# bioinfomaticsCSU/deepsignal

Hardware: AMD Instinct MI355X
Metric: CpG sites/sec (batch=512, k=17, sig=360) (higher is better)
Workload: dtype f32; 1 GPU; configs[1]: 1xMI355X, batch=512, random-init CpG model weights, synthetic (17,360) features, fp32; batch=512, kmer_len=17, signal_len=360

## Files before the change

### deepsignal_amd/csrc/ds_device.h

```cpp
#pragma once
#include "ds_internal.h"

namespace ds {

typedef float floatx16 __attribute__((ext_vector_type(16)));

__device__ __forceinline__ float4 f4max(float4 a, float4 b)
{
    return make_float4(fmaxf(a.x, b.x), fmaxf(a.y, b.y), fmaxf(a.z, b.z), fmaxf(a.w, b.w));
}
__device__ __forceinline__ float sigmoidf_(float x) { return 1.0f / (1.0f + expf(-x)); }
__device__ __forceinline__ float fast_sigmoid(float x) { return __builtin_amdgcn_rcpf(1.0f + __expf(-x)); }
__device__ __forceinline__ float fast_tanh(float x) { return fmaf(2.0f, fast_sigmoid(2.0f * x), -1.0f); }

typedef float v4f __attribute__((ext_vector_type(4)));
typedef const __attribute__((address_space(1))) v4f* gptr4;
typedef const __attribute__((address_space(1))) float* gptr1;
typedef __attribute__((address_space(1))) float* gptr1w;
__device__ __forceinline__ float4 gload4(const float* p)
{
    const v4f v = *(gptr4)(p);
    return make_float4(v.x, v.y, v.z, v.w);
}
__device__ __forceinline__ float gload(const float* p) { return *(gptr1)(p); }
__device__ __forceinline__ float4 gload4_nt(const float* p)
{
    const v4f v = __builtin_nontemporal_load((gptr4)(p));
    return make_float4(v.x, v.y, v.z, v.w);
}
__device__ __forceinline__ void gstore(float* p, float v) { *(gptr1w)(p) = v; }

typedef __bf16 bf16x8 __attribute__((ext_vector_type(8)));
__device__ __forceinline__ float bf2max(float a, float b)
{
    const unsigned ua = __float_as_uint(a), ub = __float_as_uint(b);
    const float lo = fmaxf(__uint_as_float(ua << 16), __uint_as_float(ub << 16));
    const float hi = fmaxf(__uint_as_float(ua & 0xffff0000u), __uint_as_float(ub & 0xffff0000u));
    return __uint_as_float((__float_as_uint(hi) & 0xffff0000u) | (__float_as_uint(lo) >> 16));
}
__device__ __forceinline__ float4 bf8max(float4 a, float4 b)
{
    return make_float4(bf2max(a.x, b.x), bf2max(a.y, b.y), bf2max(a.z, b.z), bf2max(a.w, b.w));
}
typedef short short2v __attribute__((ext_vector_type(2)));
__device__ __forceinline__ float bf2max_nn(float a, float b)
{
    return __builtin_bit_cast(float, __builtin_elementwise_max(__builtin_bit_cast(short2v, a), __builtin_bit_cast(short2v, b)));
}
__device__ __forceinline__ float4 bf8max_nn(float4 a, float4 b)
{
    return make_float4(bf2max_nn(a.x, b.x), bf2max_nn(a.y, b.y), bf2max_nn(a.z, b.z), bf2max_nn(a.w, b.w));
}
__device__ __forceinline__ unsigned short f2bf(float v)
{
    return __builtin_bit_cast(unsigned short, (__bf16)v);
}
__device__ __forceinline__ float bf2f(unsigned short b) { return __uint_as_float((unsigned)b << 16); }
__device__ __forceinline__ float relu_f(float x)
{
    const int b = __builtin_bit_cast(int, x);
    return __builtin_bit_cast(float, b > 0 ? b : 0);
}
typedef __bf16 bf16x2_t __attribute__((ext_vector_type(2)));
typedef float float2_t __attribute__((ext_vector_type(2)));
__device__ __forceinline__ unsigned pack_bf2(float a, float b)
{
    const float2_t f = {a, b};
    return __builtin_bit_cast(unsigned, __builtin_convertvector(f, bf16x2_t));
}

__device__ __forceinline__ floatx16 mfma_bf(float4 a, float4 b, floatx16 c)
{
    return __builtin_amdgcn_mfma_f32_32x32x16_bf16(__builtin_bit_cast(bf16x8, a), __builtin_bit_cast(bf16x8, b), c, 0, 0, 0);
}

__device__ __forceinline__ void glds16(const void* gsrc, unsigned lds_dst)
{
    unsigned keep;
    asm volatile("s_mov_b32 %0, m0\n\ts_mov_b32 m0, %2\n\ts_nop 0\n\tglobal_load_lds_dwordx4 %1, off\n\ts_mov_b32 m0, %0"
                 : "=&s"(keep)
                 : "v"(gsrc), "s"(lds_dst)
                 : "memory");
}

__device__ __forceinline__ void glds16s(const void* gbase, unsigned lane_off, unsigned lds_dst)
{
    unsigned keep;
    asm volatile("s_mov_b32 %0, m0\n\ts_mov_b32 m0, %3\n\ts_nop 0\n\tglobal_load_lds_dwordx4 %1, %2\n\ts_mov_b32 m0, %0"
// ... 82 lines not shown
```

### deepsignal_amd/csrc/ds_engine.cpp

```cpp
#include "../../include/deepsignal_hip.h"
#include "ds_internal.h"
#include "ds_extract.h"

#include <algorithm>
#include <cmath>
#include <cstdio>
#include <cstdlib>
#include <cstring>
#include <functional>
#include <map>
#include <string>
#include <vector>

using namespace ds;

namespace {

constexpr int VOCAB = 1024, EMB = 128, HID = 256, NLAYER = 3, NMOD = 11, INC_OUT = 240;
constexpr double BN_EPS = 1e-3;

thread_local std::string g_create_error;

void same_pad(int in, int k, int s, int* out, int* pl)
{
// ... 165 lines not shown

    float *stem1_w = nullptr, *stem1_b = nullptr;
    PackedGemm conv2, conv3;
    PackedGemm m_f1[NMOD];
    PackedGemm m_s1[NMOD], m_b1[NMOD], m_b3b[NMOD], m_b4b[NMOD], m_b5b[NMOD], m_b5c[NMOD];
    PackedGemm lstm_n[2][NLAYER];
    float* lstm_table[2] = {nullptr, nullptr};
    float* lstm_wfeat[2] = {nullptr, nullptr};
    PackedGemm fc1;
    float* fc2 = nullptr;
    float* w12f = nullptr;

    bool debug_keep_pool = false;
    const float* zero_seg = nullptr;
    unsigned long long* dbg_stamps = nullptr;
    unsigned long long* dbg_lstm = nullptr;
    std::vector<Stage> stages;
    KernelStat kstat[K_COUNT];
    std::vector<Slot> slots;
    Slot* cur = nullptr;
    unsigned next_slot = 0;
    int64_t plan_tick = 0;
    bool stages_done = false;
};

namespace {

int fail(ds_handle* h, int code, const std::string& msg)
{
    if (h) h->err = msg; else g_create_error = msg;
    return code;
}

#define HIPCHK(h, expr)                                                                                  \
    do {                                                                                                 \
        hipError_t e_ = (expr);                                                                          \
        if (e_ != hipSuccess) {                                                                          \
            (void)hipGetLastError();  \
            return fail(h, DS_ERR_HIP, std::string(#expr) + ": " + hipGetErrorString(e_));              \
        }                                                                                                \
    } while (0)

template <class T>
int dalloc(ds_handle* h, T** p, size_t count)
{
    void* q = nullptr;
    size_t bytes = std::max<size_t>(count * sizeof(T), 256);
    hipError_t e = hipMalloc(&q, bytes);
    if (e != hipSuccess) {
        (void)hipGetLastError();
        return fail(h, DS_ERR_NOMEM, std::string("hipMalloc: ") + hipGetErrorString(e));
    }
    h->allocs.push_back(q);
    *p = static_cast<T*>(q);
    return DS_OK;
}

int upload(ds_handle* h, float** dst, const std::vector<float>& v)
{
    int rc = dalloc(h, dst, v.size());
    if (rc) return rc;
    HIPCHK(h, hipMemcpy(*dst, v.data(), v.size() * sizeof(float), hipMemcpyHostToDevice));
    return DS_OK;
}

std::vector<float> pack_b(int K, int N, const std::function<float(int, int)>& w_in)
{
    const int Kp = (K + 31) / 32 * 32;
    auto w = [&](int k, int col) { return k < K ? w_in(k, col) : 0.0f; };
    const int ntiles = (N + 31) / 32, kg = Kp / 8;
    std::vector<float> out((size_t)ntiles * kg * 256, 0.0f);
    for (int nt = 0; nt < ntiles; ++nt)
        for (int g = 0; g < kg; ++g)
            for (int lane = 0; lane < 64; ++lane) {
                const int col = nt * 32 + (lane & 31);
                if (col >= N) continue;
                const int k0 = g * 8 + 4 * (lane >> 5);
                float* o = &out[(((size_t)nt * kg + g) * 64 + lane) * 4];
                for (int s = 0; s < 4; ++s) o[s] = w(k0 + s, col);
            }
    return out;
}

uint16_t f32_to_bf16(float f)
{
    uint32_t u;
    memcpy(&u, &f, 4);
    if ((u & 0x7fffffffu) > 0x7f800000u) return (uint16_t)((u >> 16) | 0x40);
    u += 0x7fffu + ((u >> 16) & 1);
    return (uint16_t)(u >> 16);
}

std::vector<float> pack_b_bf16(int K, int N, const std::function<float(int, int)>& w_in)
{
    const int Kp = (K + 63) / 64 * 64;
    const int ntiles = (N + 31) / 32, ks = Kp / 16;
    std::vector<uint16_t> out((size_t)ntiles * ks * 64 * 8, 0);
    for (int nt = 0; nt < ntiles; ++nt)
        for (int g = 0; g < ks; ++g)
            for (int lane = 0; lane < 64; ++lane) {
                const int col = nt * 32 + (lane & 31);
                if (col >= N) continue;
                const int k0 = g * 16 + 8 * (lane >> 5);
                uint16_t* o = &out[(((size_t)nt * ks + g) * 64 + lane) * 8];
                for (int q = 0; q < 8; ++q) o[q] = k0 + q < K ? f32_to_bf16(w_in(k0 + q, col)) : 0;
            }
    std::vector<float> raw(out.size() / 2);
    memcpy(raw.data(), out.data(), out.size() * 2);
    return raw;
}

std::vector<float> pack_b_split(int K, int N, const std::function<float(int, int)>& w_in)
{
    const int Kp = (K + 63) / 64 * 64;
    const int ntiles = (N + 31) / 32, ks = Kp / 16;
    std::vector<uint16_t> out((size_t)ntiles * ks * 3 * 64 * 8, 0);
    for (int nt = 0; nt < ntiles; ++nt)
        for (int g = 0; g < ks; ++g)
            for (int lane = 0; lane < 64; ++lane) {
                const int col = nt * 32 + (lane & 31);
                if (col >= N) continue;
                const int k0 = g * 16 + 8 * (lane >> 5);
                for (int q = 0; q < 8; ++q) {
                    if (k0 + q >= K) continue;
                    float r = w_in(k0 + q, col);
                    for (int t = 0; t < 3; ++t) {
                        const uint16_t b = f32_to_bf16(r);
                        out[((((size_t)nt * ks + g) * 3 + t) * 64 + lane) * 8 + q] = b;
                        uint32_t u = (uint32_t)b << 16;
                        float f;
                        memcpy(&f, &u, 4);
                        r -= f;
                    }
                }
            }
    std::vector<float> raw(out.size() / 2);
    memcpy(raw.data(), out.data(), out.size() * 2);
    return raw;
}

struct FoldedConv {
    int k, cin, cout;
    std::vector<float> w;
    std::vector<float> b;
};

const HostTensor* find(ds_handle* h, const std::string& name)
{
    auto it = h->host.find(name);
    return it == h->host.end() ? nullptr : &it->second;
}

int fold_conv(ds_handle* h, const std::string& scope, const std::string& conv, const std::string& bn, int k, int cin,
              int cout, FoldedConv* out)
{
    const HostTensor* ker = find(h, scope + "/" + conv + "/kernel");
    const HostTensor* beta = find(h, scope + "/" + bn + "/beta");
    const HostTensor* gamma = find(h, scope + "/" + bn + "/gamma");
    const HostTensor* mean = find(h, scope + "/" + bn + "/moving_mean");
    const HostTensor* var = find(h, scope + "/" + bn + "/moving_variance");
    if (!ker || !beta || !gamma || !mean || !var)
        return fail(h, DS_ERR_INVALID, "missing tensor(s) under " + scope + "/" + conv);
    if ((int64_t)ker->data.size() != (int64_t)k * cin * cout || (int)beta->data.size() != cout ||
        (int)gamma->data.size() != cout || (int)mean->data.size() != cout || (int)var->data.size() != cout)
        return fail(h, DS_ERR_INVALID, "bad shape for " + scope + "/" + conv + " (kernel or one of beta/gamma/moving_mean/moving_variance)");
    out->k = k; out->cin = cin; out->cout = cout;
    out->w.resize((size_t)k * cin * cout);
    out->b.resize(cout);
    std::vector<double> sc(cout);
    for (int c = 0; c < cout; ++c) {
        sc[c] = (double)gamma->data[c] / std::sqrt((double)var->data[c] + BN_EPS);
        out->b[c] = (float)((double)beta->data[c] - (double)mean->data[c] * sc[c]);
    }
    for (size_t r = 0; r < (size_t)k * cin; ++r)
        for (int c = 0; c < cout; ++c) out->w[r * cout + c] = (float)((double)ker->data[r * cout + c] * sc[c]);
    return DS_OK;
}

int upload_concat(ds_handle* h, const std::vector<const FoldedConv*>& parts, PackedGemm* pg, bool split_panel = false)
{
    const int K = parts[0]->k * parts[0]->cin;
    int N = 0;
    for (auto* p : parts) N += p->cout;
    std::vector<int> owner(N), local(N);
    int c0 = 0;
    for (size_t i = 0; i < parts.size(); ++i) {
        for (int c = 0; c < parts[i]->cout; ++c) { owner[c0 + c] = (int)i; local[c0 + c] = c; }
        c0 += parts[i]->cout;
    }
    auto wfun = [&](int k, int col) {
        const FoldedConv* p = parts[owner[col]];
        return p->w[(size_t)k * p->cout + local[col]];
    };
    std::vector<float> packed = h->bf16 ? pack_b_bf16(K, N, wfun) : pack_b(K, N, wfun);
    std::vector<float> bias((N + 31) / 32 * 32, 0.0f);
    for (int col = 0; col < N; ++col) bias[col] = parts[owner[col]]->b[local[col]];
    pg->K = h->bf16 ? (K + 1) / 2 : K; pg->N = N;
    int rc = upload(h, &pg->Bp, packed);
    if (rc) return rc;
    if (split_panel && (rc = upload(h, &pg->Bps, pack_b_split(K, N, wfun)))) return rc;
    return upload(h, &pg->bias, bias);
}

std::string mod_root(int n)
{
    char buf[128];
    snprintf(buf, sizeof buf, "modelsignalmincp_layer%d/modelsignalm%d", n, n);
    return buf;
}

int finalize_weights(ds_handle* h)
{
    int rc;
    if (h->is_cnn) {
    FoldedConv c1, c2, c3;
    if ((rc = fold_conv(h, "modelsignalmconv_layer1", "conv", "bn", 7, 1, 64, &c1))) return rc;
    if ((rc = fold_conv(h, "modelsignalmconv_layer2", "conv", "bn", 1, 64, 128, &c2))) return rc;
    if ((rc = fold_conv(h, "modelsignalmconv_layer3", "conv", "bn", 3, 128, 256, &c3))) return rc;
    if ((rc = upload(h, &h->stem1_w, c1.w))) return rc;
    if ((rc = upload(h, &h->stem1_b, c1.b))) return rc;
    if ((rc = upload_concat(h, {&c2}, &h->conv2, h->split))) return rc;
    if ((rc = upload_concat(h, {&c3}, &h->conv3, h->split))) return rc;
    for (int m = 0; m < NMOD; ++m) {
        const int cin = m == 0 ? 256 : INC_OUT;
        const std::string r = mod_root(m + 1);
        FoldedConv b1, b2, b3a, b3b, b4a, b4b, b5s, b5a, b5b, b5c;
        if ((rc = fold_conv(h, r + "branch1_maxpooling", "conv1a_1x1", "bn", 1, cin, 48, &b1))) return rc;
        if ((rc = fold_conv(h, r + "branch2_1x1", "conv0b_1x1", "bn", 1, cin, 48, &b2))) return rc;
        if ((rc = fold_conv(h, r + "branch3_1x3", "conv0c_1x1", "bn1", 1, cin, 32, &b3a))) return rc;
        if ((rc = fold_conv(h, r + "branch3_1x3", "conv1c_1x3", "bn2", 3, 32, 48, &b3b))) return rc;
        if ((rc = fold_conv(h, r + "branch4_1x5", "conv0d_1x1", "bn1", 1, cin, 32, &b4a))) return rc;
        if ((rc = fold_conv(h, r + "branch4_1x5", "conv1d_1x5", "bn2", 5, 32, 48, &b4b))) return rc;
        if ((rc = fold_conv(h, r + "branch5_residual_1x3", "convstem_1x1", "bn0", 1, cin, 48, &b5s))) return rc;
        if ((rc = fold_conv(h, r + "branch5_residual_1x3", "conv0e_1x1", "bn1", 1, cin, 32, &b5a))) return rc;
        if ((rc = fold_conv(h, r + "branch5_residual_1x3", "conv1e_1x3", "bn2", 3, 32, 64, &b5b))) return rc;
        if ((rc = fold_conv(h, r + "branch5_residual_1x3", "conv2e_1x1", "bn3", 1, 64, 48, &b5c))) return rc;
        if ((rc = upload_concat(h, {&b2, &b5s, &b3a, &b4a, &b5a}, &h->m_s1[m]))) return rc;
        if ((rc = upload_concat(h, {&b1}, &h->m_b1[m]))) return rc;
        if ((rc = upload_concat(h, {&b5s, &b2, &b3a, &b4a, &b5a, &b1}, &h->m_f1[m], h->split))) return rc;
        if ((rc = upload_concat(h, {&b3b}, &h->m_b3b[m], h->split))) return rc;
        if ((rc = upload_concat(h, {&b4b}, &h->m_b4b[m], h->split))) return rc;
        if ((rc = upload_concat(h, {&b5b}, &h->m_b5b[m], h->split))) return rc;
        if ((rc = upload_concat(h, {&b5c}, &h->m_b5c[m], h->split))) return rc;
    }
    }
    if (h->is_rnn) {
    float* d_emb = nullptr;
    if (h->is_base) {
        const HostTensor* emb = find(h, "modelembedding");
        if (!emb || (int64_t)emb->data.size() != (int64_t)VOCAB * EMB) return fail(h, DS_ERR_INVALID, "missing modelembedding");
        if ((rc = upload(h, &d_emb, emb->data))) return rc;
    }
    const int in0 = h->is_base ? EMB + 3 : 3;
    const char* dirs[2] = {"fw", "bw"};
    for (int d = 0; d < 2; ++d)
        for (int l = 0; l < NLAYER; ++l) {
            char nm[160];
            snprintf(nm, sizeof nm, "modelem/%s/multi_rnn_cell/cell_%d/lstm_cell/kernel", dirs[d], l);
            const HostTensor* ker = find(h, nm);
            snprintf(nm, sizeof nm, "modelem/%s/multi_rnn_cell/cell_%d/lstm_cell/bias", dirs[d], l);
            const HostTensor* bias = find(h, nm);
            const int in = l == 0 ? in0 : HID;
            if (!ker || !bias || (int64_t)ker->data.size() != (int64_t)(in + HID) * 4 * HID || bias->data.size() != 4 * HID)
                return fail(h, DS_ERR_INVALID, std::string("missing/bad LSTM tensor ") + nm);
            const float* kd = ker->data.data();
            const int row0 = l == 0 ? in0 : 0;
            const int K = l == 0 ? HID : 2 * HID;
            auto wfun_t = [&](int k, int pc) {
                const int p = pc / 32, i = pc % 32;
                return kd[(size_t)(row0 + k) * 4 * HID + (i >> 3) * HID + p * 8 + (i & 7)];
            };
            {
                PackedGemm& pg = h->lstm_n[d][l];
                std::function<float(int, int)> wfun = wfun_t;
                std::vector<float> packed = h->lstm_bf16 ? pack_b_bf16(K, 4 * HID, wfun) : pack_b(K, 4 * HID, wfun);
                pg.K = h->lstm_bf16 ? K / 2 : K; pg.N = 4 * HID;
                if ((rc = upload(h, &pg.Bp, packed))) return rc;
                if (h->split && (rc = upload(h, &pg.Bps, pack_b_split(K, 4 * HID, wfun)))) return rc;
                if ((rc = upload(h, &pg.bias, bias->data))) return rc;
            }
            if (l == 0) {
                if (h->is_base) {
                    float* d_k0 = nullptr;
                    std::vector<float> k0(kd, kd + (size_t)EMB * 4 * HID);
                    if ((rc = upload(h, &d_k0, k0))) return rc;
                    if ((rc = dalloc(h, &h->lstm_table[d], (size_t)VOCAB * 4 * HID))) return rc;
                    HIPCHK(h, launch_embed_table(d_emb, d_k0, h->lstm_table[d], VOCAB, EMB, 4 * HID, h->cur->s0));
                }
                std::vector<float> wf(kd + (size_t)(in0 - 3) * 4 * HID, kd + (size_t)in0 * 4 * HID);
                if ((rc = upload(h, &h->lstm_wfeat[d], wf))) return rc;
            }
        }
    }
    const HostTensor* w1 = find(h, "dense/kernel");
    const HostTensor* w2 = find(h, "dense_1/kernel");
    const int J = h->J;
    if (!w1 || !w2 || (int64_t)w1->data.size() != (int64_t)J * J || (int64_t)w2->data.size() != (int64_t)J * h->C)
        return fail(h, DS_ERR_INVALID, "missing/bad dense kernels");
    if (h->fold_fc) {
        const int C = h->C;
        std::vector<double> w12((size_t)J * C, 0.0);
        const float* a1 = w1->data.data();
        const float* a2 = w2->data.data();
        for (int k = 0; k < J; ++k) {
            double* o = &w12[(size_t)k * C];
            const float* r = a1 + (size_t)k * J;
            for (int m = 0; m < J; ++m) {
                const double v = r[m];
                for (int c = 0; c < C; ++c) o[c] += v * (double)a2[(size_t)m * C + c];
            }
        }
        const int rp = h->bf16 ? 256 : INC_OUT;
        const int ev = h->is_rnn ? 2 * HID : 0;
        std::vector<float> wf(((size_t)ev + (h->is_cnn ? (size_t)h->wc * rp : 0)) * C, 0.0f);
        for (int k = 0; k < ev; ++k)
            for (int c = 0; c < C; ++c) wf[(size_t)k * C + c] = (float)w12[(size_t)k * C + c];
        if (h->is_cnn) {
            const int wc = h->wc;
            for (int w = 0; w < wc; ++w)
                for (int ch = 0; ch < INC_OUT; ++ch)
                    for (int c = 0; c < C; ++c) {
                        double sacc = 0.0;
                        for (int wp = std::max(0, w - 3); wp <= std::min(wc - 1, w + 3); ++wp) {
                            const int cnt = std::min(wc - 1, wp + 3) - std::max(0, wp - 3) + 1;
// ... 1518 lines not shown
```

### deepsignal_amd/csrc/ds_kernels.hip

```cpp
#include "ds_device.h"

namespace ds {


template <int MT, int NT, int WM, int WN, int EPI, int AMODE, int BD, int KS, bool BF = false>
__global__ __launch_bounds__(64 * WM * WN * KS, 1) void gemm_kernel(const GemmLaunch* __restrict__ L)
{
    constexpr int BM = WM * MT * 32;
    constexpr int LDA = KC + 4;
    constexpr int NTHR = 64 * WM * WN;
    constexpr int SLOTS = (BM * 4 + NTHR - 1) / NTHR;
    constexpr int AS_FLOATS = 2 * KS * BM * LDA;
    constexpr int RED_FLOATS = KS > 1 ? WM * WN * MT * NT * 16 * 64 : 0;
    __shared__ __attribute__((aligned(16))) float smem_[AS_FLOATS > RED_FLOATS ? AS_FLOATS : RED_FLOATS];

    const int lane = threadIdx.x & 63, wave_all = __builtin_amdgcn_readfirstlane(threadIdx.x >> 6);
    const int kl = wave_all / (WM * WN);
    const int wave = wave_all % (WM * WN);
    const int tid = threadIdx.x - kl * NTHR;
    float* const As0 = smem_ + (0 * KS + kl) * BM * LDA;
    float* const As1 = smem_ + (1 * KS + kl) * BM * LDA;
    const int wm = wave % WM, wn = wave / WM;
    int bid;
    {
// ... 742 lines not shown
#pragma unroll
            for (int j = 0; j < NTW; ++j) b[j] = *reinterpret_cast<const float4*>(fb0 + SLOT * STAGE + (kgi * FR + j) * 256);
#pragma unroll
            for (int i = 0; i < MTW; ++i)
#pragma unroll
                for (int j = 0; j < NTW; ++j) acc[i][j] = mfma_bf_early(b[j], a[i], acc[i][j]);
        }
    };
    for (int st = 0; st < nstages;) {
        stage(st, LdsSlot<0>{}); if (++st >= nstages) break;
        stage(st, LdsSlot<1>{}); if (++st >= nstages) break;
        stage(st, LdsSlot<2>{}); ++st;
    }
    DS_LSTAMP(3, __builtin_amdgcn_s_memtime());

    typedef unsigned int u2v __attribute__((ext_vector_type(2)));
#pragma unroll
    for (int i = 0; i < MTW; ++i) {
        if (!valid[i]) continue;
        const int row = mt[i] * 32 + r31;
#pragma unroll
        for (int j = 0; j < NTW; ++j) {
            const int ntile = ng * FRB + nj * NTW + j;
            float4 cn, hn;
            lstm_gates(acc[i][j], cp[i][j], cn, hn);
            const v4f co = {cn.x, cn.y, cn.z, cn.w};
            *(__attribute__((address_space(1))) v4f*)(C.c + (size_t)mt[i] * LSTM_MT_FLOATS + (unsigned)ntile * 256 + lane4) = co;
            const u2v ho = {pack_bf2(hn.x, hn.y), pack_bf2(hn.z, hn.w)};
            char* const hb = reinterpret_cast<char*>(C.h_out) + (size_t)mt[i] * LSTM_MT_BYTES_BF16 + (unsigned)(ntile >> 1) * 1024 +
                             (unsigned)(((ntile & 1) * 32 + r31) * 16 + half * 8);
            *(__attribute__((address_space(1))) u2v*)hb = ho;
            if (C.h_row && row < n) {
                const v4f hr = {hn.x, hn.y, hn.z, hn.w};
                *(__attribute__((address_space(1))) v4f*)(C.h_row + (size_t)row * 256 + ntile * 8 + 4 * half) = hr;
            }
        }
    }
    DS_LSTAMP(4, __builtin_amdgcn_s_memtime());
    DS_LSTAMP(5, __builtin_amdgcn_s_memrealtime());
#undef DS_LSTAMP
}

hipError_t launch_lstm_cells(int nt, const LstmLaunch& L, hipStream_t s)
{
    const int ncell = L.ncell, mtiles = L.mtiles;
    if (ncell <= 0 || mtiles <= 0) return hipSuccess;
    const int mblocks = (mtiles + 3) / 4, mblocks2 = (mtiles + 1) / 2;
    switch (nt) {
    case 101: hipLaunchKernelGGL(lstm_cell_lds_kernel<1>, dim3(ncell * mblocks2 * 16), dim3(256), 3 * 1 * 4 * 1024, s, L); break;
    case 102: hipLaunchKernelGGL(lstm_cell_lds_kernel<2>, dim3(ncell * mblocks2 * 8), dim3(256), 3 * 2 * 6 * 1024, s, L); break;
    case 211: hipLaunchKernelGGL((lstm_cell_bf16_kernel<1, 1>), dim3(ncell * ((mtiles + 1) / 2) * 16), dim3(256), 3 * 2 * 4 * 1024, s, L); break;
    case 212: hipLaunchKernelGGL((lstm_cell_bf16_kernel<1, 2>), dim3(ncell * ((mtiles + 1) / 2) * 8), dim3(256), 3 * 2 * 6 * 1024, s, L); break;
    case 222: hipLaunchKernelGGL((lstm_cell_bf16_kernel<2, 2>), dim3(ncell * ((mtiles + 3) / 4) * 8), dim3(256), 3 * 2 * 8 * 1024, s, L); break;
    case 1: hipLaunchKernelGGL(lstm_cell_kernel<1>, dim3(ncell * mblocks * 32), dim3(256), 0, s, L); break;
    case 2: hipLaunchKernelGGL(lstm_cell_kernel<2>, dim3(ncell * mblocks * 16), dim3(256), 0, s, L); break;
    case 4: hipLaunchKernelGGL(lstm_cell_kernel<4>, dim3(ncell * mblocks * 8), dim3(256), 0, s, L); break;
    default: return hipErrorInvalidValue;
    }
    return hipGetLastError();
}

#ifndef DS_FUSED_WPS
#define DS_FUSED_WPS 2
#endif
#ifndef DS_FUSED_BD
#define DS_FUSED_BD 2
#endif
#ifndef DS_FUSED_POOLPRIO
#define DS_FUSED_POOLPRIO 0
#endif
#ifndef DS_FUSED_VD
#define DS_FUSED_VD 2
#endif
constexpr int F_LDA = KC + 4;
constexpr int F_LD1 = 100;
constexpr int F_LD2 = 68;

size_t inception_fused_lds_bytes(int tm, int W, int spt)
{
    const int tr32 = tm * 32;
    return (size_t)(tr32 * F_LD1 + (spt * (W + 4) + 5) * F_LD1 + tr32 * F_LD2 + tr32 + 192) * sizeof(float);
}

__device__ __forceinline__ void fused_unit_prefetch(const float* __restrict__ Bp, int ntaps, int nt, int lane, float4 (&ub)[20])
{
    const float* bsrc = Bp + ((size_t)(nt * ntaps * 4) * 64 + lane) * 4;
#pragma unroll
    for (int g = 0; g < 20; ++g)
        if (g < ntaps * 4) ub[g] = gload4(bsrc + g * 256);
}

template <int NTAPS>
__device__ __forceinline__ void fused_conv_unit(const float* T1, int rm, int coloff, int lane, const float4 (&ub)[20], floatx16& acc)
{
    const float* base = T1 + rm * F_LD1 + coloff + (lane >> 5) * 4;
#pragma unroll
    for (int t = 0; t < NTAPS; ++t) {
        const float* arow = base + (t - NTAPS / 2) * F_LD1;
#pragma unroll
        for (int g = 0; g < 4; ++g) {
            const float4 a = *reinterpret_cast<const float4*>(arow + g * 8);
            acc = __builtin_amdgcn_mfma_f32_32x32x2f32(ub[t * 4 + g].x, a.x, acc, 0, 0, 0);
            acc = __builtin_amdgcn_mfma_f32_32x32x2f32(ub[t * 4 + g].y, a.y, acc, 0, 0, 0);
            acc = __builtin_amdgcn_mfma_f32_32x32x2f32(ub[t * 4 + g].z, a.z, acc, 0, 0, 0);
            acc = __builtin_amdgcn_mfma_f32_32x32x2f32(ub[t * 4 + g].w, a.w, acc, 0, 0, 0);
        }
    }
}

struct FusedTagT { static constexpr bool value = true; };
struct FusedTagF { static constexpr bool value = false; };

template <int TM>
__device__ __forceinline__ void inception_fused_body(const FusedChain& c)
{
    constexpr int TR32 = TM * 32;
    extern __shared__ __attribute__((aligned(16))) float smem[];
    float* Ad = smem;
    float* Ys = smem;
    float* T1 = smem + TR32 * F_LD1;
    const int W = c.m[0].W, spt = c.m[0].spt;
    float* T2 = T1 + (spt * (W + 4) + 5) * F_LD1;
    int* rowmap = reinterpret_cast<int*>(T2 + TR32 * F_LD2);
    float* const Bs = reinterpret_cast<float*>(rowmap + TR32);
    const int site0 = blockIdx.x * spt;
    const int nhere = min(spt, c.m[0].n_sites - site0);
    const int TRv = nhere * W;
    const size_t grow0 = (size_t)site0 * W;
    for (int i = threadIdx.x; i < (spt * (W + 4) + 5) * (F_LD1 / 4); i += 512)
        reinterpret_cast<float4*>(T1)[i] = make_float4(0.f, 0.f, 0.f, 0.f);
    if (threadIdx.x < TR32)
        rowmap[threadIdx.x] = (int)threadIdx.x < TRv ? ((int)threadIdx.x / W) * (W + 4) + 2 + (int)threadIdx.x % W : spt * (W + 4) + 2;

    for (int mi = 0; mi < c.nmod; ++mi) {
    const FusedArgs& a = c.m[mi];
    int tid_opaque = threadIdx.x, wave_opaque = __builtin_amdgcn_readfirstlane(threadIdx.x >> 6);
    asm volatile("" : "+v"(tid_opaque), "+s"(wave_opaque));
    const int tid = tid_opaque, lane = tid & 63, wave = wave_opaque;
    const int cin = a.cin;
    const gptr1w Yg = (gptr1w)(a.Y + grow0 * 240);

    const bool stamp = a.dbg != nullptr && lane == 0 && (wave == 0 || wave == 7) && blockIdx.x < DBG_MAX_WGS;
#define DS_STAMP(i) do { if (stamp) (a.dbg + ((size_t)blockIdx.x * 2 + (wave == 7)) * 8)[i] = __builtin_amdgcn_s_memtime(); } while (0)
    DS_STAMP(0);
    if (tid >= 256 && tid < 448) {
        const int q = tid - 256;
        Bs[q] = gload((q < 64 ? a.bias5b : q < 128 ? a.bias3b : a.bias4b) + (q & 63));
    }

    const bool stager = tid < TR32 * 4;
    const int sr = tid >> 2, sq = tid & 3;
    const int rr = sr < TRv ? sr : TRv - 1;
    const bool pooled_in = a.pool_win > 0;
    const float *pc, *pq = nullptr, *pr = nullptr;
    if (!pooled_in) {
        pc = a.X + (grow0 + rr) * cin + sq * 4;
    } else {
        const int s_ = rr / W, w_ = rr % W;
        const int i0 = 2 * w_ - a.pool_pad;
        const int ia = i0 < 0 ? i0 + 1 : i0;
        const int ib = i0 + 1 < a.pool_win ? (i0 + 1 < 0 ? ia : i0 + 1) : ia;
        const int ic = i0 + 2 < a.pool_win ? i0 + 2 : ib;
        const float* sb = a.X + ((size_t)(site0 + s_) * a.pool_win) * cin + sq * 4;
        pc = sb + (size_t)ia * cin;
        pq = sb + (size_t)ib * cin;
        pr = sb + (size_t)ic * cin;
    }
    const float* bp = a.Bp1 + ((size_t)wave * ((cin + 31) / 32 * 4) * 64 + lane) * 4;

    const int h4 = 4 * (lane >> 5), rlane = lane & 31;
    floatx16 acc[TM];
    {
        float4 bv[4];
#pragma unroll
        for (int g = 0; g < 4; ++g) {
            bv[g] = gload4(a.bias1 + wave * 32 + 8 * g + h4);
            if (wave < 2) {
                const float4 t = gload4(a.bias5c + wave * 32 + 8 * g + h4);
                bv[g].x += t.x; bv[g].y += t.y; bv[g].z += t.z; bv[g].w += t.w;
            }
        }
#pragma unroll
        for (int mt = 0; mt < TM; ++mt)
#pragma unroll
            for (int g = 0; g < 4; ++g) {
                acc[mt][4 * g + 0] = bv[g].x; acc[mt][4 * g + 1] = bv[g].y;
                acc[mt][4 * g + 2] = bv[g].z; acc[mt][4 * g + 3] = bv[g].w;
            }
    }

    int offm[TM], offp[TM];
// ... 9 lines not shown

    __builtin_assume(nchunks >= 15 && nchunks <= 16);
    auto run_p1 = [&](auto pool_tag) {
        constexpr bool POOL = decltype(pool_tag)::value;
        constexpr int VD = DS_FUSED_VD;
        float4 vc[VD];
        constexpr int BD = DS_FUSED_BD;
        float4 bq[BD][2];
        float4 af[2][2][TM];
        auto load_a = [&](int V) __attribute__((always_inline)) {
            if (!POOL && stager) {
                vc[V] = gload4(pc); pc += KC;
                if (pooled_in) {
                    vc[V] = f4max(f4max(vc[V], gload4(pq)), gload4(pr));
                    pq += KC; pr += KC;
                }
            }
        };
        auto store_a = [&](int X, int V) __attribute__((always_inline)) {
            if (!POOL && stager) *reinterpret_cast<float4*>(Ad + X * TR32 * F_LDA + sr * F_LDA + sq * 4) = vc[V];
        };
        auto load_b = [&](int Bi) __attribute__((always_inline)) {
            bq[Bi][0] = gload4(bp);
            bq[Bi][1] = gload4(bp + 256);
            bp += 512;
        };
        auto read_frags = [&](int X) __attribute__((always_inline)) {
#pragma unroll
            for (int rs = 0; rs < 2; ++rs)
#pragma unroll
                for (int mt = 0; mt < TM; ++mt) {
                    const float* q = Ad + X * TR32 * F_LDA + (mt * 32 + (lane & 31)) * F_LDA + rs * 8 + (lane >> 5) * 4;
                    float4 v = *reinterpret_cast<const float4*>(q);
                    if (POOL) v = f4max(f4max(v, *reinterpret_cast<const float4*>(q + offm[mt])), *reinterpret_cast<const float4*>(q + offp[mt]));
                    af[X][rs][mt] = v;
                }
        };
        auto mfma_rs = [&](int X, int Bi, int rs) __attribute__((always_inline)) {
#pragma unroll
            for (int mt = 0; mt < TM; ++mt) {
                acc[mt] = __builtin_amdgcn_mfma_f32_32x32x2f32(bq[Bi][rs].x, af[X][rs][mt].x, acc[mt], 0, 0, 0);
                acc[mt] = __builtin_amdgcn_mfma_f32_32x32x2f32(bq[Bi][rs].y, af[X][rs][mt].y, acc[mt], 0, 0, 0);
                acc[mt] = __builtin_amdgcn_mfma_f32_32x32x2f32(bq[Bi][rs].z, af[X][rs][mt].z, acc[mt], 0, 0, 0);
                acc[mt] = __builtin_amdgcn_mfma_f32_32x32x2f32(bq[Bi][rs].w, af[X][rs][mt].w, acc[mt], 0, 0, 0);
            }
        };
#pragma unroll
        for (int i = 0; i < VD; ++i) load_a(i);
#pragma unroll
        for (int i = 0; i < BD - 1; ++i) load_b(i);
        store_a(0, 0);
        __syncthreads();
        read_frags(0);
#pragma unroll
        for (int c = 0; c < 16; ++c) {
            if (c < nchunks) {
                const int X = c & 1;
                const bool has1 = c + 1 < nchunks;
                if (c + VD < nchunks) load_a(c % VD);
                if (c + BD - 1 < nchunks) load_b((c + BD - 1) % BD);
                if (has1) store_a(X ^ 1, (c + 1) % VD);
                mfma_rs(X, c % BD, 0);
                __builtin_amdgcn_sched_barrier(0);
                __syncthreads();
                if (has1) read_frags(X ^ 1);
                mfma_rs(X, c % BD, 1);
                __builtin_amdgcn_sched_group_barrier(0x8, 1, 0);
                if (has1) __builtin_amdgcn_sched_group_barrier(0x100, (POOL ? 6 : 2) * TM, 0);
                __builtin_amdgcn_sched_group_barrier(0x8, 4 * TM, 0);
                __builtin_amdgcn_sched_barrier(0);
            }
        }
    };
    if (wave >= 6) { __builtin_amdgcn_s_setprio(DS_FUSED_POOLPRIO); run_p1(FusedTagT{}); __builtin_amdgcn_s_setprio(0); }
    else run_p1(FusedTagF{});
    DS_STAMP(1);
    __syncthreads();
    DS_STAMP(2);

    int a1k = 0, a1m = 0, a1n = 0, a2k = 0, a2m = 0, a2n = 0;
    int b1k = 0, b1m = 0, b1n = 0, b2k = 0, b2m = 0, b2n = 0;
    if (TM == 3) {
        if (wave < 6) { a1k = 1; a1m = wave % 3; a1n = wave / 3; }
        else { a1k = 2; a1m = 0; a1n = wave - 6; }
        if (wave >= 2) { b1k = 3; b1m = (wave - 2) % 3; b1n = (wave - 2) / 3; }
        if (wave >= 4) { b2k = 2; b2m = 1 + ((wave - 4) >> 1); b2n = (wave - 4) & 1; }
    } else if (TM == 2) {
        if (wave < 4) { a1k = 1; a1m = wave & 1; a1n = wave >> 1; }
        else { a1k = 2; a1m = wave & 1; a1n = (wave - 4) >> 1; }
        if (wave >= 2 && wave < 6) { b1k = 3; b1m = (wave - 2) & 1; b1n = (wave - 2) >> 1; }
    } else {
        if (wave < 2) { a1k = 1; a1n = wave; }
        else if (wave < 4) { a1k = 2; a1n = wave - 2; }
        else if (wave < 6) { a1k = 3; a1n = wave - 4; }
    }
    auto unit_Bp = [&](int k) { return k == 1 ? a.Bp5b : k == 2 ? a.Bp3b : a.Bp4b; };
    auto unit_taps = [&](int k) { return k == 3 ? 5 : 3; };
    float4 pf[20];
#pragma unroll
    for (int g = 0; g < 20; ++g) pf[g] = make_float4(0.f, 0.f, 0.f, 0.f);
    if (a1k) fused_unit_prefetch(unit_Bp(a1k), unit_taps(a1k), a1n, lane, pf);

    if (wave >= 3 && wave <= 5) {
#pragma unroll
        for (int mt = 0; mt < TM; ++mt) {
            const int rm = rowmap[mt * 32 + rlane];
#pragma unroll
            for (int g = 0; g < 4; ++g)
                *reinterpret_cast<float4*>(T1 + rm * F_LD1 + (wave * 32 - 96) + 8 * g + h4) =
                    make_float4(relu_f(acc[mt][4 * g]), relu_f(acc[mt][4 * g + 1]), relu_f(acc[mt][4 * g + 2]),
                                relu_f(acc[mt][4 * g + 3]));
        }
    } else if (wave != 0) {
#pragma unroll
        for (int g = 0; g < 4; ++g) {
            const int col = wave * 32 + 8 * g + h4;
            if (col >= 48 && col < 240) {
                const int ycol = col < 96 ? col : col - 192;
#pragma unroll
                for (int mt = 0; mt < TM; ++mt)
                    *reinterpret_cast<float4*>(Ys + (mt * 32 + rlane) * F_LD1 + ycol) =
                        make_float4(relu_f(acc[mt][4 * g]), relu_f(acc[mt][4 * g + 1]), relu_f(acc[mt][4 * g + 2]),
                                    relu_f(acc[mt][4 * g + 3]));
            }
        }
    }
    DS_STAMP(3);
    __syncthreads();
    DS_STAMP(4);
    for (int idx = tid; idx < TR32 * 24; idx += 512) {
        const int row = idx / 24, q = idx - row * 24;
        if (row < TRv) {
            const float4 v = *reinterpret_cast<const float4*>(Ys + row * F_LD1 + q * 4);
            v4f o = {v.x, v.y, v.z, v.w};
            *(__attribute__((address_space(1))) v4f*)(Yg + (unsigned)(row * 240 + q * 4)) = o;
        }
    }

    auto run_unit = [&](int kind, int mt, int nt) {
        floatx16 u;
        const float* bsrc = Bs + (kind == 1 ? 0 : kind == 2 ? 64 : 128) + nt * 32 + h4;
#pragma unroll
        for (int g = 0; g < 4; ++g) {
            const float4 t = *reinterpret_cast<const float4*>(bsrc + 8 * g);
            u[4 * g] = t.x; u[4 * g + 1] = t.y; u[4 * g + 2] = t.z; u[4 * g + 3] = t.w;
        }
        const int row = mt * 32 + rlane;
        const int rm = rowmap[row];
        if (kind == 1) {
            fused_conv_unit<3>(T1, rm, 64, lane, pf, u);
#pragma unroll
            for (int g = 0; g < 4; ++g)
                *reinterpret_cast<float4*>(T2 + row * F_LD2 + nt * 32 + 8 * g + h4) =
                    make_float4(relu_f(u[4 * g]), relu_f(u[4 * g + 1]), relu_f(u[4 * g + 2]), relu_f(u[4 * g + 3]));
        } else {
            if (kind == 2) fused_conv_unit<3>(T1, rm, 0, lane, pf, u);
            else fused_conv_unit<5>(T1, rm, 32, lane, pf, u);
            const int ybase = kind == 2 ? 96 : 144;
            if (row < TRv) {
#pragma unroll
                for (int g = 0; g < 4; ++g)
                    if (nt * 32 + 8 * g < 48) {
                        v4f o = {relu_f(u[4 * g]), relu_f(u[4 * g + 1]), relu_f(u[4 * g + 2]), relu_f(u[4 * g + 3])};
                        *(__attribute__((address_space(1))) v4f*)(Yg + (unsigned)(row * 240 + ybase + nt * 32 + 8 * g + h4)) = o;
                    }
            }
        }
    };

    if (a1k) run_unit(a1k, a1m, a1n);
    if (a2k) {
        fused_unit_prefetch(unit_Bp(a2k), unit_taps(a2k), a2n, lane, pf);
        run_unit(a2k, a2m, a2n);
    }
    float4 b5c[8];
#pragma unroll
    for (int g = 0; g < 8; ++g) b5c[g] = make_float4(0.f, 0.f, 0.f, 0.f);
    if (wave < 2) {
#pragma unroll
        for (int g = 0; g < 8; ++g) b5c[g] = gload4(a.Bp5c + ((size_t)(wave * 8 + g) * 64 + lane) * 4);
    } else if (b1k) {
        fused_unit_prefetch(unit_Bp(b1k), unit_taps(b1k), b1n, lane, pf);
    }
    DS_STAMP(5);
    __syncthreads();
    DS_STAMP(6);

    if (wave < 2) {
#pragma unroll
        for (int mt = 0; mt < TM; ++mt) {
            const float* base = T2 + (mt * 32 + rlane) * F_LD2 + h4;
#pragma unroll
            for (int g = 0; g < 8; ++g) {
                const float4 av = *reinterpret_cast<const float4*>(base + g * 8);
                acc[mt] = __builtin_amdgcn_mfma_f32_32x32x2f32(b5c[g].x, av.x, acc[mt], 0, 0, 0);
                acc[mt] = __builtin_amdgcn_mfma_f32_32x32x2f32(b5c[g].y, av.y, acc[mt], 0, 0, 0);
                acc[mt] = __builtin_amdgcn_mfma_f32_32x32x2f32(b5c[g].z, av.z, acc[mt], 0, 0, 0);
                acc[mt] = __builtin_amdgcn_mfma_f32_32x32x2f32(b5c[g].w, av.w, acc[mt], 0, 0, 0);
            }
        }
#pragma unroll
        for (int mt = 0; mt < TM; ++mt) {
            const int row = mt * 32 + rlane;
            if (row < TRv) {
#pragma unroll
                for (int g = 0; g < 4; ++g)
                    if (wave * 32 + 8 * g < 48) {
                        v4f o = {relu_f(acc[mt][4 * g]), relu_f(acc[mt][4 * g + 1]), relu_f(acc[mt][4 * g + 2]),
                                 relu_f(acc[mt][4 * g + 3])};
                        *(__attribute__((address_space(1))) v4f*)(Yg + (unsigned)(row * 240 + 192 + wave * 32 + 8 * g + h4)) = o;
                    }
            }
        }
    } else {
        if (b1k) run_unit(b1k, b1m, b1n);
        if (b2k) {
            fused_unit_prefetch(unit_Bp(b2k), unit_taps(b2k), b2n, lane, pf);
            run_unit(b2k, b2m, b2n);
        }
    }
    DS_STAMP(7);
#undef DS_STAMP
    if (mi + 1 < c.nmod) __syncthreads();
    }
}

template <int TM>
__global__ __launch_bounds__(512, DS_FUSED_WPS) void inception_fused_kernel(const FusedChain c) { inception_fused_body<TM>(c); }
static bool fused_chain_ok(const FusedChain& c)
{
    if (c.nmod <= 0 || c.nmod > FUSED_CHAIN_MAX) return false;
    for (int i = 1; i < c.nmod; ++i)
        if (c.m[i].W != c.m[0].W || c.m[i].spt != c.m[0].spt || c.m[i].n_sites != c.m[0].n_sites || c.m[i].pool_win != 0 ||
            c.m[i].X != c.m[i - 1].Y) return false;
    return true;
}

hipError_t launch_inception_fused(int tm, const FusedChain& c, hipStream_t s)
{
    if (!fused_chain_ok(c)) return hipErrorInvalidValue;
    const FusedArgs& a = c.m[0];
    if (a.n_sites <= 0) return hipSuccess;
    for (int i = 0; i < c.nmod; ++i)
        if (c.m[i].cin != 240 && c.m[i].cin != 256) return hipErrorInvalidValue;
    const size_t lds = inception_fused_lds_bytes(tm, a.W, a.spt);
    const int grid = (a.n_sites + a.spt - 1) / a.spt;
    switch (tm) {
    case 1: hipLaunchKernelGGL(inception_fused_kernel<1>, dim3(grid), dim3(512), lds, s, c); break;
    case 2: hipLaunchKernelGGL(inception_fused_kernel<2>, dim3(grid), dim3(512), lds, s, c); break;
    case 3: hipLaunchKernelGGL(inception_fused_kernel<3>, dim3(grid), dim3(512), lds, s, c); break;
    default: return hipErrorInvalidValue;
    }
    return hipGetLastError();
}

#ifndef DS_FUSEDB_WPS
#define DS_FUSEDB_WPS 4
#endif
#ifndef DS_FUSEDB_NT
#define DS_FUSEDB_NT 1
#endif
#if DS_FUSEDB_NT
#define DS_FUSEDB_TILE_LOAD(p) gload4_nt(p)
#else
#define DS_FUSEDB_TILE_LOAD(p) gload4(p)
#endif
#ifndef DS_FUSEDB_POOLPRIO
#define DS_FUSEDB_POOLPRIO 2
#endif
#ifndef DS_FUSEDB_RING
#define DS_FUSEDB_RING 2
#endif
constexpr int B_LDA = 132;
constexpr int B_LD1 = 52;

size_t inception_fused_bf16_lds_bytes(int tm, int W, int spt)
{
    const int tr32 = tm * 32;
    return (size_t)(tr32 * B_LDA + (spt * (W + 4) + 5) * B_LD1 + tr32 + 192) * sizeof(float);
}

__device__ __forceinline__ void fusedb_unit_prefetch(const float* __restrict__ Bp, int ntaps, int nt, int lane, float4 (&ub)[10])
{
    const int ks = (ntaps * 32 + 63) / 64 * 4;
    const float* bsrc = Bp + ((size_t)(nt * ks) * 64 + lane) * 4;
#pragma unroll
    for (int g = 0; g < 10; ++g)
        if (g < ntaps * 2) ub[g] = gload4(bsrc + g * 256);
}

template <int NTAPS>
__device__ __forceinline__ void fusedb_conv_unit(const float* T1, int rm, int coloff_units, int lane, const float4 (&ub)[10], floatx16& acc)
{
    const float* base = T1 + rm * B_LD1 + coloff_units + (lane >> 5) * 4;
#pragma unroll
    for (int t = 0; t < NTAPS; ++t) {
        const float* arow = base + (t - NTAPS / 2) * B_LD1;
#pragma unroll
        for (int j = 0; j < 2; ++j)
            acc = mfma_bf(ub[t * 2 + j], *reinterpret_cast<const float4*>(arow + j * 8), acc);
    }
// ... 1065 lines not shown
```

Before: 416,100 sites/s.

## Use 16-wide MFMA tiles for 48-column conv tails and rebalance wave units

The b3b/b4b convolution branches have 48 output columns, so the second 32-wide MFMA tile previously computed 16 wasted columns. A packed 16-column B tail is now uploaded, and those tail units use 16x16x4 f32 MFMAs over two 16-row halves instead of a padded 32x32 tile. The TM=3 wave-to-unit assignment is reshuffled to balance the now-cheaper tail units. Each call slot is also specialised at compile time to the unit kinds it can see, which cuts code size and register pressure. This adds weight-packing complexity and changes the MFMA shape, which may shift the accumulator layout and register use.

```diff
diff --git a/deepsignal_amd/csrc/ds_device.h b/deepsignal_amd/csrc/ds_device.h
--- a/deepsignal_amd/csrc/ds_device.h
+++ b/deepsignal_amd/csrc/ds_device.h
@@ -4,6 +4,7 @@
 namespace ds {
 
 typedef float floatx16 __attribute__((ext_vector_type(16)));
+typedef float floatx4 __attribute__((ext_vector_type(4)));
 
 __device__ __forceinline__ float4 f4max(float4 a, float4 b)
 {
diff --git a/deepsignal_amd/csrc/ds_engine.cpp b/deepsignal_amd/csrc/ds_engine.cpp
--- a/deepsignal_amd/csrc/ds_engine.cpp
+++ b/deepsignal_amd/csrc/ds_engine.cpp
@@ -271,6 +271,17 @@
     return out;
 }
 
+std::vector<float> pack_b_n16(int K, int col0, const std::function<float(int, int)>& w)
+{
+    const int kg = K / 16;
+    std::vector<float> out((size_t)kg * 256, 0.0f);
+    for (int g = 0; g < kg; ++g)
+        for (int lane = 0; lane < 64; ++lane)
+            for (int s = 0; s < 4; ++s)
+                out[((size_t)g * 64 + lane) * 4 + s] = w(g * 16 + 4 * (lane >> 4) + s, col0 + (lane & 15));
+    return out;
+}
+
 uint16_t f32_to_bf16(float f)
 {
     uint32_t u;
@@ -366,7 +377,7 @@
     return DS_OK;
 }
 
-int upload_concat(ds_handle* h, const std::vector<const FoldedConv*>& parts, PackedGemm* pg, bool split_panel = false)
+int upload_concat(ds_handle* h, const std::vector<const FoldedConv*>& parts, PackedGemm* pg, bool split_panel = false, bool n16_tail = false)
 {
     const int K = parts[0]->k * parts[0]->cin;
     int N = 0;
@@ -382,6 +393,11 @@
         return p->w[(size_t)k * p->cout + local[col]];
     };
     std::vector<float> packed = h->bf16 ? pack_b_bf16(K, N, wfun) : pack_b(K, N, wfun);
+    if (n16_tail && !h->bf16) {
+        if (N != 48 || K % 32) return fail(h, DS_ERR_INVALID, "n16_tail: a [32 t x 48] operand expected");
+        const std::vector<float> t = pack_b_n16(K, 32, wfun);
+        packed.insert(packed.end(), t.begin(), t.end());
+    }
     std::vector<float> bias((N + 31) / 32 * 32, 0.0f);
     for (int col = 0; col < N; ++col) bias[col] = parts[owner[col]]->b[local[col]];
     pg->K = h->bf16 ? (K + 1) / 2 : K; pg->N = N;
@@ -427,8 +443,8 @@
         if ((rc = upload_concat(h, {&b2, &b5s, &b3a, &b4a, &b5a}, &h->m_s1[m]))) return rc;
         if ((rc = upload_concat(h, {&b1}, &h->m_b1[m]))) return rc;
         if ((rc = upload_concat(h, {&b5s, &b2, &b3a, &b4a, &b5a, &b1}, &h->m_f1[m], h->split))) return rc;
-        if ((rc = upload_concat(h, {&b3b}, &h->m_b3b[m], h->split))) return rc;
-        if ((rc = upload_concat(h, {&b4b}, &h->m_b4b[m], h->split))) return rc;
+        if ((rc = upload_concat(h, {&b3b}, &h->m_b3b[m], h->split, true))) return rc;
+        if ((rc = upload_concat(h, {&b4b}, &h->m_b4b[m], h->split, true))) return rc;
         if ((rc = upload_concat(h, {&b5b}, &h->m_b5b[m], h->split))) return rc;
         if ((rc = upload_concat(h, {&b5c}, &h->m_b5c[m], h->split))) return rc;
     }
diff --git a/deepsignal_amd/csrc/ds_kernels.hip b/deepsignal_amd/csrc/ds_kernels.hip
--- a/deepsignal_amd/csrc/ds_kernels.hip
+++ b/deepsignal_amd/csrc/ds_kernels.hip
@@ -848,12 +848,13 @@
     return (size_t)(tr32 * F_LD1 + (spt * (W + 4) + 5) * F_LD1 + tr32 * F_LD2 + tr32 + 192) * sizeof(float);
 }
 
-__device__ __forceinline__ void fused_unit_prefetch(const float* __restrict__ Bp, int ntaps, int nt, int lane, float4 (&ub)[20])
-{
-    const float* bsrc = Bp + ((size_t)(nt * ntaps * 4) * 64 + lane) * 4;
+__device__ __forceinline__ void fused_unit_prefetch(const float* __restrict__ Bp, int ntaps, int nt, bool n16, int lane, float4 (&ub)[20])
+{
+    const float* bsrc = Bp + ((size_t)((n16 ? 2 : nt) * ntaps * 4) * 64 + lane) * 4;
+    const int cnt = n16 ? ntaps * 2 : ntaps * 4;
 #pragma unroll
     for (int g = 0; g < 20; ++g)
-        if (g < ntaps * 4) ub[g] = gload4(bsrc + g * 256);
+        if (g < cnt) ub[g] = gload4(bsrc + g * 256);
 }
 
 template <int NTAPS>
@@ -873,6 +874,35 @@
         }
     }
 }
+
+template <int NTAPS>
+__device__ __forceinline__ void fused_conv_unit16(const float* T1, int rm0, int rm1, int coloff, int lane, const float4 (&ub)[20],
+                                                  floatx4& acc0, floatx4& acc1)
+{
+    const int ko = coloff + (lane >> 4) * 4;
+#pragma unroll
+    for (int t = 0; t < NTAPS; ++t) {
+        const float* r0 = T1 + (rm0 + t - NTAPS / 2) * F_LD1 + ko;
+        const float* r1 = T1 + (rm1 + t - NTAPS / 2) * F_LD1 + ko;
+#pragma unroll
+        for (int g = 0; g < 2; ++g) {
+            const float4 a0 = *reinterpret_cast<const float4*>(r0 + g * 16);
+            const float4 a1 = *reinterpret_cast<const float4*>(r1 + g * 16);
+            const float4 b = ub[t * 2 + g];
+            acc0 = __builtin_amdgcn_mfma_f32_16x16x4f32(b.x, a0.x, acc0, 0, 0, 0);
+            acc1 = __builtin_amdgcn_mfma_f32_16x16x4f32(b.x, a1.x, acc1, 0, 0, 0);
+            acc0 = __builtin_amdgcn_mfma_f32_16x16x4f32(b.y, a0.y, acc0, 0, 0, 0);
+            acc1 = __builtin_amdgcn_mfma_f32_16x16x4f32(b.y, a1.y, acc1, 0, 0, 0);
+            acc0 = __builtin_amdgcn_mfma_f32_16x16x4f32(b.z, a0.z, acc0, 0, 0, 0);
+            acc1 = __builtin_amdgcn_mfma_f32_16x16x4f32(b.z, a1.z, acc1, 0, 0, 0);
+            acc0 = __builtin_amdgcn_mfma_f32_16x16x4f32(b.w, a0.w, acc0, 0, 0, 0);
+            acc1 = __builtin_amdgcn_mfma_f32_16x16x4f32(b.w, a1.w, acc1, 0, 0, 0);
+        }
+    }
+}
+
+constexpr int FU_B5B = 1, FU_B3B = 2, FU_B4B = 4, FU_B3B16 = 8, FU_B4B16 = 16;
+template <int M> struct FusedUnits { static constexpr int value = M; };
 
 struct FusedTagT { static constexpr bool value = true; };
 struct FusedTagF { static constexpr bool value = false; };
@@ -1048,9 +1078,10 @@
     int b1k = 0, b1m = 0, b1n = 0, b2k = 0, b2m = 0, b2n = 0;
     if (TM == 3) {
         if (wave < 6) { a1k = 1; a1m = wave % 3; a1n = wave / 3; }
-        else { a1k = 2; a1m = 0; a1n = wave - 6; }
-        if (wave >= 2) { b1k = 3; b1m = (wave - 2) % 3; b1n = (wave - 2) / 3; }
-        if (wave >= 4) { b2k = 2; b2m = 1 + ((wave - 4) >> 1); b2n = (wave - 4) & 1; }
+        else { a1k = 2; a1m = wave - 6; a1n = 0; }
+        if (wave >= 2) { b1k = 3; b1m = wave == 2 || wave == 4 ? 0 : wave == 3 || wave == 5 ? 1 : 2; b1n = wave == 4 || wave == 5 || wave == 7; }
+        if (wave == 2 || wave == 7) { b2k = 2; b2m = 2; b2n = wave == 2; }
+        if (wave == 4 || wave == 5) { b2k = 2; b2m = wave - 4; b2n = 1; }
     } else if (TM == 2) {
         if (wave < 4) { a1k = 1; a1m = wave & 1; a1n = wave >> 1; }
         else { a1k = 2; a1m = wave & 1; a1n = (wave - 4) >> 1; }
@@ -1065,7 +1096,8 @@
     float4 pf[20];
 #pragma unroll
     for (int g = 0; g < 20; ++g) pf[g] = make_float4(0.f, 0.f, 0.f, 0.f);
-    if (a1k) fused_unit_prefetch(unit_Bp(a1k), unit_taps(a1k), a1n, lane, pf);
+    auto unit_prefetch = [&](int k, int n) { fused_unit_prefetch(unit_Bp(k), unit_taps(k), n, k >= 2 && n == 1, lane, pf); };
+    if (a1k) unit_prefetch(a1k, a1n);
 
     if (wave >= 3 && wave <= 5) {
 #pragma unroll
@@ -1103,9 +1135,35 @@
         }
     }
 
-    auto run_unit = [&](int kind, int mt, int nt) {
+    auto run_unit = [&](auto forms_tag, int kind, int mt, int nt) {
+        constexpr int FORMS = decltype(forms_tag)::value;
+        const int boff = kind == 1 ? 0 : kind == 2 ? 64 : 128;
+        if (kind >= 2 && nt == 1) {
+            if constexpr ((FORMS & (FU_B3B16 | FU_B4B16)) != 0) {
+                const int q4 = 4 * (lane >> 4);
+                const float4 t = *reinterpret_cast<const float4*>(Bs + boff + 32 + q4);
+                floatx4 u0 = {t.x, t.y, t.z, t.w}, u1 = u0;
+                const int row0 = mt * 32 + (lane & 15), row1 = row0 + 16;
+                const int rm0 = rowmap[row0], rm1 = rowmap[row1];
+                if (kind == 2) {
+                    if constexpr ((FORMS & FU_B3B16) != 0) fused_conv_unit16<3>(T1, rm0, rm1, 0, lane, pf, u0, u1);
+                } else {
+                    if constexpr ((FORMS & FU_B4B16) != 0) fused_conv_unit16<5>(T1, rm0, rm1, 32, lane, pf, u0, u1);
+                }
+                const int ycol = (kind == 2 ? 96 : 144) + 32 + q4;
+                if (row0 < TRv) {
+                    v4f o = {relu_f(u0[0]), relu_f(u0[1]), relu_f(u0[2]), relu_f(u0[3])};
+                    *(__attribute__((address_space(1))) v4f*)(Yg + (unsigned)(row0 * 240 + ycol)) = o;
+                }
+                if (row1 < TRv) {
+                    v4f o = {relu_f(u1[0]), relu_f(u1[1]), relu_f(u1[2]), relu_f(u1[3])};
+                    *(__attribute__((address_space(1))) v4f*)(Yg + (unsigned)(row1 * 240 + ycol)) = o;
+                }
+            }
+            return;
+        }
         floatx16 u;
-        const float* bsrc = Bs + (kind == 1 ? 0 : kind == 2 ? 64 : 128) + nt * 32 + h4;
+        const float* bsrc = Bs + boff + nt * 32 + h4;
 #pragma unroll
         for (int g = 0; g < 4; ++g) {
             const float4 t = *reinterpret_cast<const float4*>(bsrc + 8 * g);
@@ -1114,30 +1172,39 @@
         const int row = mt * 32 + rlane;
         const int rm = rowmap[row];
         if (kind == 1) {
-            fused_conv_unit<3>(T1, rm, 64, lane, pf, u);
-#pragma unroll
-            for (int g = 0; g < 4; ++g)
-                *reinterpret_cast<float4*>(T2 + row * F_LD2 + nt * 32 + 8 * g + h4) =
-                    make_float4(relu_f(u[4 * g]), relu_f(u[4 * g + 1]), relu_f(u[4 * g + 2]), relu_f(u[4 * g + 3]));
-        } else {
-            if (kind == 2) fused_conv_unit<3>(T1, rm, 0, lane, pf, u);
-            else fused_conv_unit<5>(T1, rm, 32, lane, pf, u);
+            if constexpr ((FORMS & FU_B5B) != 0) {
+                fused_conv_unit<3>(T1, rm, 64, lane, pf, u);
+#pragma unroll
+                for (int g = 0; g < 4; ++g)
+                    *reinterpret_cast<float4*>(T2 + row * F_LD2 + nt * 32 + 8 * g + h4) =
+                        make_float4(relu_f(u[4 * g]), relu_f(u[4 * g + 1]), relu_f(u[4 * g + 2]), relu_f(u[4 * g + 3]));
+            }
+        } else if constexpr ((FORMS & (FU_B3B | FU_B4B)) != 0) {
+            if (kind == 2) {
+                if constexpr ((FORMS & FU_B3B) != 0) fused_conv_unit<3>(T1, rm, 0, lane, pf, u);
+            } else {
+                if constexpr ((FORMS & FU_B4B) != 0) fused_conv_unit<5>(T1, rm, 32, lane, pf, u);
+            }
             const int ybase = kind == 2 ? 96 : 144;
             if (row < TRv) {
 #pragma unroll
-                for (int g = 0; g < 4; ++g)
-                    if (nt * 32 + 8 * g < 48) {
-                        v4f o = {relu_f(u[4 * g]), relu_f(u[4 * g + 1]), relu_f(u[4 * g + 2]), relu_f(u[4 * g + 3])};
-                        *(__attribute__((address_space(1))) v4f*)(Yg + (unsigned)(row * 240 + ybase + nt * 32 + 8 * g + h4)) = o;
-                    }
+                for (int g = 0; g < 4; ++g) {
+                    v4f o = {relu_f(u[4 * g]), relu_f(u[4 * g + 1]), relu_f(u[4 * g + 2]), relu_f(u[4 * g + 3])};
+                    *(__attribute__((address_space(1))) v4f*)(Yg + (unsigned)(row * 240 + ybase + 8 * g + h4)) = o;
+                }
             }
         }
     };
-
-    if (a1k) run_unit(a1k, a1m, a1n);
+    constexpr int ALLF = FU_B5B | FU_B3B | FU_B4B | FU_B3B16 | FU_B4B16;
+    using SlotA1 = FusedUnits<TM == 3 ? (FU_B5B | FU_B3B) : ALLF>;
+    using SlotA2 = FusedUnits<TM == 3 ? 0 : ALLF>;
+    using SlotB1 = FusedUnits<TM == 3 ? (FU_B4B | FU_B4B16) : ALLF>;
+    using SlotB2 = FusedUnits<TM == 3 ? (FU_B3B | FU_B3B16) : ALLF>;
+
+    if (a1k) run_unit(SlotA1{}, a1k, a1m, a1n);
     if (a2k) {
-        fused_unit_prefetch(unit_Bp(a2k), unit_taps(a2k), a2n, lane, pf);
-        run_unit(a2k, a2m, a2n);
+        unit_prefetch(a2k, a2n);
+        run_unit(SlotA2{}, a2k, a2m, a2n);
     }
     float4 b5c[8];
 #pragma unroll
@@ -1146,7 +1213,7 @@
 #pragma unroll
         for (int g = 0; g < 8; ++g) b5c[g] = gload4(a.Bp5c + ((size_t)(wave * 8 + g) * 64 + lane) * 4);
     } else if (b1k) {
-        fused_unit_prefetch(unit_Bp(b1k), unit_taps(b1k), b1n, lane, pf);
+        unit_prefetch(b1k, b1n);
     }
     DS_STAMP(5);
     __syncthreads();
@@ -1179,10 +1246,10 @@
             }
         }
     } else {
-        if (b1k) run_unit(b1k, b1m, b1n);
+        if (b1k) run_unit(SlotB1{}, b1k, b1m, b1n);
         if (b2k) {
-            fused_unit_prefetch(unit_Bp(b2k), unit_taps(b2k), b2n, lane, pf);
-            run_unit(b2k, b2m, b2n);
+            unit_prefetch(b2k, b2n);
+            run_unit(SlotB2{}, b2k, b2m, b2n);
         }
     }
     DS_STAMP(7);
```

Result: faster. 420,900 sites/s (median of 6 runs) (+1.1%).
